# danielzgtg/TTS.cpp

Measured on AMD Instinct MI355X. Metric: audio-sec/wall-sec (RTF^-1), Parler-TTS-mini v1 Q4_K AR decode + DAC decode, higher is better.
Workload: dtype q4_K weights x q8_K activations (int dot, f32 combine); DAC f16 im2col x f32 weights, f64 accumulate

## Files before the change

### include/tts_hip.h

```cpp
#ifndef TTS_HIP_H
#define TTS_HIP_H

#include <stddef.h>
#include <stdint.h>

#ifdef __cplusplus
extern "C" {
#endif

#define TTS_MAX_DIMS 4
#define TTS_MAX_SRC 4
#define TTS_MAX_OP_PARAMS 16
#define TTS_MAX_NAME 64

enum tts_type {
    TTS_TYPE_F32 = 0,
    TTS_TYPE_F16 = 1,
    TTS_TYPE_Q4_0 = 2,
    TTS_TYPE_Q4_1 = 3,
    TTS_TYPE_Q5_0 = 6,
    TTS_TYPE_Q5_1 = 7,
    TTS_TYPE_Q8_0 = 8,
    TTS_TYPE_Q8_1 = 9,
    TTS_TYPE_Q4_K = 12,
// ... 168 lines not shown
    TTS_HIP_OPT_ATTN_PV16 = 15,
    TTS_HIP_OPT_GEMV_PREQUANT = 21,
    TTS_HIP_OPT_GEMV_KRELAY = 22,
    TTS_HIP_OPT_ATTN_KS = 23,
    TTS_HIP_OPT_ATTN_PV8 = 24,
    TTS_HIP_OPT_GEMV_KRELAY_LOOP = 26,
    TTS_HIP_OPT_GEMV_Q80_PRO = 27,
    TTS_HIP_OPT_GEMV_Q80_SLAB = 28,
    TTS_HIP_OPT_GEMV_Q80_RW = 29,
    TTS_HIP_OPT_GEMM_Q8_STAGED = 30,
    TTS_HIP_OPT_GEMV_KR_INKERNEL = 31,
    TTS_HIP_OPT_GEMV_F32_WIDE = 32,
    TTS_HIP_OPT_ATTN_PV_MP = 33,
    TTS_HIP_OPT_GEMM_KR_INKERNEL = 35,
    TTS_HIP_OPT_GEMM_KR_CT2 = 36,
    TTS_HIP_OPT_GEMM_KR_NW = 34,
    TTS_HIP_OPT_GEMV_NW_MIN = 25,
    TTS_HIP_OPT_GEMM_KR_XCD = 38,
    TTS_HIP_OPT_GEMM_KR_CP = 39,
    TTS_HIP_OPT_GEMM_KR_WALK = 40,
    TTS_HIP_OPT_GEMM_PF = 41,
    TTS_HIP_OPT_GEMM_PF_NW = 42,
    TTS_HIP_OPT_ATTN_ONE = 43,
    TTS_HIP_OPT_COALESCE = 37,
};
enum tts_fuse_bits {
    TTS_FUSE_LN = 1, TTS_FUSE_GROUP = 2, TTS_FUSE_KV = 4, TTS_FUSE_EPI = 8, TTS_FUSE_HEADS = 16, TTS_FUSE_ATTN = 32,
    TTS_FUSE_LSTM = 64,
    TTS_FUSE_SNAKE = 128,
    TTS_FUSE_EMBED = 256,
    TTS_FUSE_CONV = 512,
    TTS_FUSE_ADAIN = 1024,
    TTS_FUSE_XATTN = 2048,
    TTS_FUSE_MCPY = 4096,
    TTS_FUSE_CONTREAD = 8192
};
int tts_hip_set_option(tts_hip_backend_t backend, int option, int value);
int tts_hip_attn_decode(tts_hip_backend_t backend, const tts_tensor * q, const tts_tensor * k, const tts_tensor * v,
                        const float * mask, int64_t mbs, float scale, float * out, float * out2, const int64_t * koff,
                        const int64_t * voff, const int64_t * moff, const int32_t * pseq);
int tts_hip_coalesce_stats(int device, int64_t * out, int n);
void tts_hip_coalesce_set_wait(int us);
int tts_hip_coalesce_enable(int on);
#define TTS_HIP_HOOK_FAULT_WEIGHT_SET 1
int tts_hip_test_hook(int hook, int value);
int tts_hip_install_crash_handler(void);
// ... 3 lines not shown
typedef struct tts_sampling {
    float temperature;
    float top_p;
    float repetition_penalty;
    int32_t top_k;
    int32_t do_sample;
    int32_t pad_;
    uint64_t seed;
} tts_sampling;
void tts_sampling_default(tts_sampling * cfg);
uint32_t tts_sampler_call_seed(uint64_t seed, int32_t stream, int64_t call);
int tts_sampler_sample(const tts_sampling * cfg, const float * logits, int32_t NH, int32_t V, uint32_t call_seed, int32_t * last,
                       int32_t * count, int32_t * out);
int tts_hip_sample_step(tts_hip_backend_t backend, const float * logits, int32_t B, int32_t NH, int32_t V, const tts_sampling * cfg,
                        int64_t call, int32_t * rep_state, int32_t step, int32_t bos, int32_t eos, int32_t * eos_seen, int32_t * hist,
                        int32_t * next);
int tts_sampling_device_ok(const tts_sampling * cfg, int32_t V);
int tts_hip_counters(tts_hip_backend_t backend, int64_t * out, int n);

int tts_hip_gemv(tts_hip_backend_t backend, int type, const void * w, const float * x, float * y,
                 int64_t K, int64_t N, int64_t M);
int tts_hip_gemv_ex(tts_hip_backend_t backend, int type, const void * w, const float * x, float * y,
                    int64_t K, int64_t N, int64_t M, int32_t wflags);

typedef struct tts_backend_iface {
    void * ctx;
    const char * name;
    void * (*alloc)(void * ctx, size_t size);
    void (*free)(void * ctx, void * ptr);
    int (*set)(void * ctx, void * dst, const void * src, size_t size);
    int (*set_tensor)(void * ctx, tts_tensor * t, const void * src);
    int (*get)(void * ctx, void * dst, const void * src, size_t size);
    int (*memset)(void * ctx, void * dst, int value, size_t size);
    int (*compute)(void * ctx, tts_tensor * const * nodes, int n_nodes);
    int (*synchronize)(void * ctx);
    int (*prepare)(void * ctx, tts_tensor * const * nodes, int n_nodes, int slot);
    int (*launch)(void * ctx, int slot);
    int (*set_async)(void * ctx, void * dst, const void * src, size_t size);
    int (*copy)(void * ctx, void * dst, const void * src, size_t size);
    int (*greedy_step)(void * ctx, const float * logits, int B, int NH, int V, int step, int bos, int eos, int32_t * eos_seen,
                       int32_t * hist, int32_t * next);
    int (*sample_step)(void * ctx, const float * logits, int B, int NH, int V, const tts_sampling * cfg, int64_t call, int32_t * rep_state,
                       int step, int bos, int eos, int32_t * eos_seen, int32_t * hist, int32_t * next);
} tts_backend_iface;

int tts_hip_backend_iface(tts_hip_backend_t backend, tts_backend_iface * out);
// ... 7 lines not shown
```

### tts.cpp_amd/csrc/backend.hip

```cpp
#include <cmath>
#include <atomic>
#include <cstring>
#include <map>
#include <mutex>
#include <thread>

#include "hip_internal.h"
#include <hip/hip_ext.h>

#include <dlfcn.h>
#include <execinfo.h>
#include <fcntl.h>
#include <signal.h>
#include <unistd.h>

using namespace tts;


static void build_gelu_table(uint16_t * t) {
    const float GELU_COEF_A = 0.044715f;
    const float SQRT_2_OVER_PI = 0.79788456080286535587989211986876f;
    for (int i = 0; i < 65536; ++i) {
        const float x = fp16_to_fp32_host((uint16_t)i);
        const float g = 0.5f * x * (1.0f + tanhf(SQRT_2_OVER_PI * x * (1.0f + GELU_COEF_A * x * x)));
// ... 716 lines not shown
        case TTS_HIP_OPT_GEMV_Q80_SLAB: be->gemv_q80_slab = value != 0; return 0;
        case TTS_HIP_OPT_GEMV_KR_INKERNEL:
            if (value < 0) return TTS_STATUS_BAD_ARG;
            be->gemv_kr_ink = value;
            return 0;
        case TTS_HIP_OPT_GEMM_Q8_STAGED:
            if (value < 0 || value > 2) return TTS_STATUS_BAD_ARG;
            be->gemm_q8_staged = value;
            return 0;
        case TTS_HIP_OPT_GEMV_Q80_RW:
            if (value < 0 || value > 32 || (value & (value - 1))) return TTS_STATUS_BAD_ARG;
            be->gemv_q80_rw = value;
            return 0;
        case TTS_HIP_OPT_ATTN_KS: be->attn_ks = value; return 0;
        case TTS_HIP_OPT_GEMV_NW_MIN: be->gemv_nw_min = value; return 0;
        case TTS_HIP_OPT_ATTN_PV8: be->attn_pv8 = value != 0; return 0;
        case TTS_HIP_OPT_GEMM_KR_CT2: be->gemm_kr_ct2 = value != 0; return 0;
        case TTS_HIP_OPT_GEMM_KR_INKERNEL: be->gemm_kr_ink = value < 0 ? 0 : value; return 0;
        case TTS_HIP_OPT_ATTN_PV_MP: be->attn_pv_mp = value == 2 ? 2 : value != 0; return 0;
        case TTS_HIP_OPT_ATTN_ONE:
            if (value < 0 || value > 2) return TTS_STATUS_BAD_ARG;
            be->attn_one = value;
            return 0;
        case TTS_HIP_OPT_GEMM_KR_NW: be->gemm_kr_nw = value == 8 ? 8 : 4; return 0;
        case TTS_HIP_OPT_GEMM_Q8: be->gemm_q8 = value != 0; return 0;
        case TTS_HIP_OPT_CU_PARTITION: {
            const int count = value & 0xFF, index = (value >> 8) & 0xFF;
            const bool inter = (value >> 16) & 1;
            hipSetDevice(be->device);
            TTS_HIP_CHECK(hipStreamSynchronize(be->stream));
            hipStream_t ns = nullptr;
            if (count <= 1) {
                TTS_HIP_CHECK(hipStreamCreateWithFlags(&ns, hipStreamNonBlocking));
                be->cus = be->cu_total;
            } else {
                if (index >= count) return TTS_STATUS_BAD_ARG;
                std::vector<uint32_t> mask((be->cu_total + 31) / 32, 0u);
                const int per = be->cu_total / count;
                int n = 0;
                for (int c = 0; c < be->cu_total; ++c) {
                    const bool on = inter ? (c % count == index) : (c / per == index && c < per * count);
                    if (on) mask[c / 32] |= 1u << (c % 32), ++n;
                }
                if (hipExtStreamCreateWithCUMask(&ns, (uint32_t)mask.size(), mask.data()) != hipSuccess) return TTS_STATUS_FAILED;
                be->cus = n;
            }
// ... 113 lines not shown
```

### tts.cpp_amd/csrc/coalesce.hip

```cpp
#include <algorithm>
#include <atomic>
#include <chrono>
#include <condition_variable>
#include <cstring>
#include <map>
#include <mutex>
#include <thread>
#include <unordered_map>
#include <unordered_set>

#include "hip_internal.h"

namespace tts {
namespace {

using Clock = std::chrono::steady_clock;

struct Req {
    tts_hip_backend * be = nullptr;
    tts_tensor * const * nodes = nullptr;
    int n = 0;
    uint64_t sig = 0;
    int64_t count = 0;
    bool taken = false, done = false;
// ... 134 lines not shown
            for (int d = 0; d < 4; ++d) mix((uint64_t)t->src[0]->ne[d]);
    }
    return (h ^ (h2 * 0x94D049BB133111EBull)) | 1;
}

void copy_options(tts_hip_backend * d, const tts_hip_backend * s) {
    d->fusion = s->fusion;
    d->attn_split_minp = s->attn_split_minp;
    d->attn_ks = s->attn_ks;
    d->attn_pv_mp = s->attn_pv_mp;
    d->attn_one = s->attn_one;
    d->attn_pv8 = s->attn_pv8;
    d->attn_pv_uv16 = s->attn_pv_uv16;
    d->attn_fused_minp = s->attn_fused_minp;
    d->gemv_unique = s->gemv_unique;
    d->gemm_q8 = s->gemm_q8;
    d->bgemm_f32 = s->bgemm_f32;
    d->gemv_f32_wide = s->gemv_f32_wide;
    d->gemm_kr_nw = s->gemm_kr_nw;
    d->gemv_ks_tiles = s->gemv_ks_tiles;
    d->gemv_mf_prequant = s->gemv_mf_prequant;
    d->gemv_kr = s->gemv_kr;
    d->gemv_kr_loop = s->gemv_kr_loop;
    d->gemv_q80_pro = s->gemv_q80_pro;
    d->gemv_q80_slab = s->gemv_q80_slab;
    d->gemv_q80_rw = s->gemv_q80_rw;
    d->gemm_q8_staged = s->gemm_q8_staged;
    d->gemv_kr_ink = s->gemv_kr_ink;
    d->gemm_kr_ct2 = s->gemm_kr_ct2;
    d->gemm_kr_xcd = s->gemm_kr_xcd;
    d->gemm_kr_cp = s->gemm_kr_cp;
    d->gemm_kr_ink = s->gemm_kr_ink;
    d->gemv_nw_min = s->gemv_nw_min;
    d->gemv_mf_rsplit = s->gemv_mf_rsplit;
    d->profile_gemv = s->profile_gemv;
}

__global__ void k_ne_bytes(const uint4 * __restrict__ a, const uint4 * __restrict__ b, size_t n16, const uint8_t * __restrict__ ta,
                           const uint8_t * __restrict__ tb, size_t tail, int * flag) {
    bool ne = false;
    for (size_t i = (size_t)blockIdx.x * blockDim.x + threadIdx.x; i < n16; i += (size_t)gridDim.x * blockDim.x) {
        const uint4 x = a[i], y = b[i];
        ne |= x.x != y.x || x.y != y.y || x.z != y.z || x.w != y.w;
    }
    if (blockIdx.x == 0)
        for (size_t i = threadIdx.x; i < tail; i += blockDim.x) ne |= ta[i] != tb[i];
// ... 362 lines not shown
```

### tts.cpp_amd/csrc/graph_exec.hip

```cpp
#include <algorithm>
#include <cstring>
#include <deque>
#include <unordered_map>
#include <vector>

#include <array>

#include "hip_internal.h"
#include <chrono>

using namespace tts;

namespace tts {
void launch_kv_prefetch(tts_hip_backend * be, hipStream_t st, const TD & t, int pdim, int blocks);
void launch_gemv_q4K_xattn(tts_hip_backend * be, const GemvJob & j, const XAttnArgs & a);
void launch_attn_decode(tts_hip_backend * be, const TD & q, const TD & k, const TD & v, const float * mask, float scale,
                        float * out, int hd, int P, int H, int n, int B, float * out2, int64_t obs = -1, int64_t mbs = 0,
                        const int64_t * koff = nullptr, const int64_t * voff = nullptr, const int64_t * moff = nullptr,
                        const int * pseq = nullptr);
void launch_layernorm(tts_hip_backend * be, const tts_tensor * dst, const tts_tensor * x, const float * w, const float * b,
                      float eps, bool rms);
}

namespace {
// ... 2820 lines not shown
            if (!keep) be->aq.src = nullptr;
        }
    }
    if (pf_pending >= 0) TTS_HIP_CHECK(hipStreamWaitEvent(be->stream, be->pf_join, 0));
    if (be->bat) {
        if (n_sc > 0) {
            hipLaunchKernelGGL(k_co_scatter, dim3(4, (unsigned)n_sc), dim3(256), 0, be->stream, (const int64_t *)be->co_tab + sc_off, n_sc);
            TTS_HIP_CHECK(hipGetLastError());
            co_readback(be, sc_host, n_sc);
        }
        be->bat->comap = nullptr;
    }
    return 0;
}
}

extern "C" int tts_hip_gemv(tts_hip_backend_t be, int type, const void * w, const float * x, float * y, int64_t K, int64_t N,
                            int64_t M) {
    return tts_hip_gemv_ex(be, type, w, x, y, K, N, M, 0);
}

extern "C" int tts_hip_gemv_ex(tts_hip_backend_t be, int type, const void * w, const float * x, float * y, int64_t K, int64_t N,
                               int64_t M, int32_t wflags) {
    if (!be) return TTS_STATUS_BAD_ARG;
    if ((wflags & TTS_FLAG_TILED) && (type != TTS_TYPE_Q4_K || N % 4)) return TTS_STATUS_BAD_ARG;
    if (type == TTS_TYPE_Q4_K && K % 256) return TTS_STATUS_BAD_ARG;
    if (type == TTS_TYPE_Q8_0 && K % 32) return TTS_STATUS_BAD_ARG;
    if (type != TTS_TYPE_Q4_K && type != TTS_TYPE_Q8_0 && type != TTS_TYPE_F16 && type != TTS_TYPE_F32) return TTS_STATUS_UNSUPPORTED;
    if ((type == TTS_TYPE_F32 || type == TTS_TYPE_F16) && K % 4) return TTS_STATUS_BAD_ARG;
    hipSetDevice(be->device);
    GemvJob j;
    j.wtype = type;
    j.K = K;
    j.N = N;
    j.M = M;
    j.w_row_bytes = (int64_t)tts_row_size(type, K);
    j.W[0] = (const uint8_t *)w;
    j.Y[0] = y;
    j.ycs[0] = N;
    j.yrs[0] = 1;
    j.x = x;
    j.xcs = K;
    const bool q80pro = type == TTS_TYPE_Q8_0 && K % QK_K == 0 && M <= 8 && be->gemv_q80_pro;
    if (type == TTS_TYPE_Q4_K || q80pro) {
        j.pro = PRO_QUANT;
        j.tiled = (wflags & TTS_FLAG_TILED) ? 1 : 0;
        if ((uintptr_t)x & 15) {
            if ((size_t)(4 * K * M) > be->scratch_size) return TTS_STATUS_ALLOC_FAILED;
            launch_copy_cols(be, (float *)be->scratch, x, K, K, M);
            be->aq.src = nullptr;
            j.x = (const float *)be->scratch;
        }
    } else if (type != TTS_TYPE_F32) {
        if (act_quant_bytes(type, K, M) > be->scratch_size) return TTS_STATUS_ALLOC_FAILED;
        launch_quantize_act(be, type, x, K, K, M, j.aq);
    } else {
        j.aq.vtype = TTS_TYPE_F32;
    }
    be->aq.src = nullptr;
    launch_gemv_job(be, j);
    return 0;
}
```

### tts.cpp_amd/csrc/hip_internal.h

```cpp
#pragma once

#include <hip/hip_fp16.h>
#include <hip/hip_runtime.h>

#include <cstdio>
#include <cstdlib>
#include <atomic>
#include <deque>
#include <mutex>
#include <unordered_map>
#include <tuple>
#include <vector>

#include "common.h"

#define TTS_HIP_CHECK(expr)                                                                          \
    do {                                                                                             \
        hipError_t err_ = (expr);                                                                    \
        if (err_ != hipSuccess) {                                                                    \
            fprintf(stderr, "%s:%d: HIP error %s: %s\n", __FILE__, __LINE__, #expr, hipGetErrorString(err_)); \
            abort();                                                                                 \
        }                                                                                            \
    } while (0)

// ... 151 lines not shown
    int64_t xcs = 0;
    ActQuant aq;
    int pro = 0;
    int tiled = 0;
    int hetero = 0;
    int64_t roff[GEMV_MAX_MATS + 1] = {};
    int32_t rep_mat = -1, yrg = 0, nrep = 0;
    int64_t yrgs = 0, yrep = 0;
    int dbg = 0;
    const float * lnw = nullptr;
    const float * lnb = nullptr;
    float eps = 0.f;
    int rms = 0;
    float * lnout = nullptr;
    int64_t locs = 0;
    const char * bq = nullptr;
    int64_t bq_bytes = 0;
    int64_t bq_tile = 0;
    int32_t bq_slot = 0;
    unsigned long long * ts = nullptr;
    const int64_t * yoff = nullptr;
    int32_t yoff_mats = 0, yoff_ld = 0;
    int32_t xcd_cols = 0;
};
__host__ __device__ inline int64_t job_roff(const GemvJob & j, int m) { return j.hetero ? j.roff[m] : (int64_t)m * j.N; }
__host__ __device__ inline int64_t job_rows(const GemvJob & j) { return job_roff(j, j.nmat); }
#ifdef TTS_PHASE_TS
#define TTS_TS(job, k)                                                                                            \
    do {                                                                                                          \
        if ((job).ts && (threadIdx.x & 63) == 0)                                                                  \
            (job).ts[((((size_t)blockIdx.z * gridDim.y + blockIdx.y) * gridDim.x + blockIdx.x) * (blockDim.x >> 6) + \
                      (threadIdx.x >> 6)) * 8 +                                                                   \
                     (k)] = __builtin_amdgcn_s_memrealtime();                                                     \
    } while (0)
#else
#define TTS_TS(job, k) \
    do {               \
    } while (0)
#endif
enum { PRO_QUANT = 1, PRO_LN = 2, PRO_COPY = 3 };
struct XAttnArgs {
    TD k, v;
    const float * mask = nullptr;
    float scale = 1.f;
    float * out = nullptr;
    float * out2 = nullptr;
    int P = 0, H = 0, B = 0;
// ... 78 lines not shown
    size_t attn_floats = 0;
    int attn_split_minp = 128;
    int attn_ks = 2;
    int attn_pv_mp = 1;
    int attn_one = 1;
    int attn_pv8 = 0;
    int attn_pv_uv16 = 0;
    int attn_fused_minp = 0;
    unsigned long long * argmax_keys = nullptr;
    unsigned * argmax_counts = nullptr;
    int64_t q4k_tile_bytes = 4 << 20;
    int gemv_dbg = 0;
    int gemv_unique = 1;
    int gemm_q8 = 1;
    int64_t cus = 256;
    int cu_total = 256;
    int bgemm_f32 = 1;
    int gemv_f32_wide = 1;
    int gemm_kr_nw = 4;
    int64_t gemv_ks_tiles = 256;
    int gemv_mf_prequant = 1;
    int gemv_kr = 1;
    int gemv_kr_loop = 1;
    int gemv_q80_pro = 1;
    int gemv_q80_slab = 1;
    int gemv_q80_rw = 0;
    int gemm_q8_staged = 2;
    int64_t gemv_kr_ink = 0;
    int gemm_kr_walk = 0;
    int gemm_pf = 64;
    int gemm_pf_nw = 4;
    int gemm_kr_cp = 0;
    int gemm_kr_xcd = 0;
    int gemm_kr_ct2 = 0;
    int64_t gemm_kr_ink = 0;
    int gemv_nw_min = 0;
    int gemv_mf_rsplit = 1;
    int64_t q4k_dual_bytes = 1 << 20;
    void * sample_cand = nullptr;
    size_t sample_cand_size = 0;
    int kv_prefetch_minp = 0;
    int kv_prefetch_blocks = 128;
    hipStream_t pf_stream = nullptr;
    hipEvent_t pf_fork = nullptr, pf_join = nullptr;
    uint8_t * pin = nullptr;
    size_t pin_size = 0, pin_head = 0;
// ... 189 lines not shown
```

### tts.cpp_amd/csrc/k_gemv.hip

```cpp
#include "hip_internal.h"
#include <hip/hip_ext.h>

#include <atomic>
#include <type_traits>

#ifndef TTS_GEMV_EARLY16
#define TTS_GEMV_EARLY16 1
#endif

namespace tts {

__device__ __forceinline__ float dev_fp16_to_fp32(uint16_t h) {
    return __half2float(__ushort_as_half(h));
}

__device__ __forceinline__ int dev_nearest_int(float f) {
    const float val = __fadd_rn(f, 12582912.f);
    const int i = __float_as_int(val);
    return (i & 0x007fffff) - 0x00400000;
}

__global__ __launch_bounds__(256) void k_quantize_q8_K(const float * __restrict__ x, int64_t xcs, int64_t K,
                                                       int8_t * __restrict__ qs, float * __restrict__ dout,
                                                       int32_t * __restrict__ s32) {
// ... 83 lines not shown
    const int m = blockIdx.y;
    const int64_t i = (int64_t)blockIdx.x * blockDim.x + threadIdx.x;
    if (i < K) out[m * K + i] = __float2half_rn(x[m * xcs + i]);
}

__device__ __forceinline__ void q4k_scale_min(const uint8_t * q, int j, int & sc, int & mn) {
    if (j < 4) {
        sc = q[j] & 63;
        mn = q[j + 4] & 63;
    } else {
        sc = (q[j + 4] & 0xF) | ((q[j - 4] >> 6) << 4);
        mn = (q[j + 4] >> 4) | ((q[j] >> 6) << 4);
    }
}

__device__ __forceinline__ size_t al16(size_t n) { return (n + 15) & ~(size_t)15; }

__device__ __forceinline__ int xcd_contiguous(int b, int n) {
    const int x = b & 7, q = n >> 3, r = n & 7;
    return x * q + (x < r ? x : r) + (b >> 3);
}


template <int MC>
__device__ __forceinline__ void gemv_store(const GemvJob & j, int mat, int64_t row, int m, float v) {
    if (j.epi == EPI_GELU) {
        if (v <= -10.0f) v = 0.0f;
        else if (v < 10.0f) v = __half2float(__ushort_as_half(j.gelu[__half_as_ushort(__float2half_rn(v))]));
    } else if (j.epi == EPI_ADD) {
        v = __fadd_rn(v, j.res[m * j.rcs + row]);
    } else if (j.epi == EPI_SILU_MUL) {
        v = __fmul_rn(dev_silu(j.res[m * j.rcs + row]), v);
    }
    float * const Y = j.Y[mat] + ((j.yoff_mats >> mat) & 1 ? j.yoff[mat * j.yoff_ld + m] : 0);
    const int64_t ycs = j.ycs[mat], yrs = j.yrs[mat];
    if (mat == j.rep_mat) {
        const int64_t g = row / j.yrg;
        float * y = Y + m * ycs + g * j.yrgs + (row - g * j.yrg) * yrs;
        for (int k = 0; k < j.nrep; ++k) y[k * j.yrep] = v;
        return;
    }
    Y[m * ycs + row * yrs] = v;
}

__device__ __forceinline__ void q8k_quant16(const float (&v)[16], int lane, int (&q)[16], float & d, int & s) {
    float lax = 0.f, lval = 0.f;
#pragma unroll
    for (int e = 0; e < 16; ++e) {
        const float a = fabsf(v[e]);
        const bool gt = a > lax;
        lax = gt ? a : lax;
        lval = gt ? v[e] : lval;
    }
    unsigned mx = __float_as_uint(lax);
    mx = max(mx, (unsigned)dpp_i32<DPP_XOR1>((int)mx));
    mx = max(mx, (unsigned)dpp_i32<DPP_XOR2>((int)mx));
// ... 844 lines not shown
                    qb[bf][u][l] = ld((const uint32_t *)(bp + 16 + (l + 4) * 16 + kg * 4));
                }
            }
        } else {
            const uint8_t * wt = j.W[mat] + (row >> 2) * nb * 576;
            const int ri = (int)(row & 3);
#pragma unroll
            for (int u = 0; u < BPW; ++u) {
                const uint8_t * bp = wt + (int64_t)min(w * BPW + u, nb - 1) * 576;
                hd[bf][u] = ld((const u32x4 *)(bp + ri * 16));
                qa[bf][u] = ld((const u32x4 *)(bp + 64 + ((kg * 2) * 4 + ri) * 16));
                qb[bf][u] = ld((const u32x4 *)(bp + 64 + ((kg * 2 + 1) * 4 + ri) * 16));
            }
        }
        TTS_PIN_LOADS();
    };
    auto load_w = [&](auto BUF, int64_t t) __attribute__((always_inline)) {
        if (!LOOP && CTW == 1 && j.xcd_cols && gridDim.y > 1) load_w_pol(BUF, std::true_type{}, t);
        else load_w_pol(BUF, std::false_type{}, t);
    };
    using B0 = std::integral_constant<int, 0>;
    using B1 = std::integral_constant<int, LOOP ? 1 : 0>;
    int64_t t = tx;
    if constexpr (PRO == PRO_COPY) {
        const int nck = (int)((ntile * bqb) >> 10);
        for (int i = wave; i < nck; i += nw)
            __builtin_amdgcn_global_load_lds(gptr(bqt + (size_t)i * 1024 + lane * 16),
                                             (__attribute__((address_space(3))) void *)(smem + (size_t)i * 1024), 16, 0, 0);
        TTS_PIN_LOADS();
        load_w(B0{}, t);
    } else {
        auto first = [&]() __attribute__((always_inline)) { load_w(B0{}, t); };
        ProOv ov;
        ov.col0 = c0;
        ov.mcols = M;
        q4k_prologue<PRO, 16, true, decltype(first)>(j, nb, nullptr, xd_s, nullptr, b16, sbs, first, ov);
    }
    TTS_TS(j, 1);
    __syncthreads();
    TTS_TS(j, 2);

    f2v tp[BPW][8][2], tq[BPW][2];
    auto terms = [&](auto BUF) __attribute__((always_inline)) {
        constexpr int bf = decltype(BUF)::value;
#pragma unroll
        for (int u = 0; u < BPW; ++u) {
            const int b = min(w * BPW + u, nb - 1);
            const u32x4 h = hd[bf][u];
            const uint32_t sc_lo = h.y & 0x3F3F3F3Fu, mn_lo = h.z & 0x3F3F3F3Fu;
            const uint32_t sc_hi = (h.w & 0x0F0F0F0Fu) | ((h.y >> 2) & 0x30303030u);
            const uint32_t mn_hi = ((h.w >> 4) & 0x0F0F0F0Fu) | ((h.z >> 2) & 0x30303030u);
            const uint32_t sw = (kg < 2 ? sc_lo : sc_hi) >> ((kg & 1) * 16);
            const _Float16 s0 = (_Float16)(float)(sw & 0xFF), s1 = (_Float16)(float)((sw >> 8) & 0xFF);
            const f16x2 S0 = {s0, s0}, S1 = {s1, s1};
            const _Float16 o0 = (_Float16)(-1024.f * (float)(sw & 0xFF)), o1 = (_Float16)(-1024.f * (float)((sw >> 8) & 0xFF));
// ... 87 lines not shown
        float tot[4];
        if (w == nwt - 1) {
#pragma unroll
            for (int q = 0; q < 4; ++q) {
                tot[q] = sumf[q >> 1][q & 1];
#pragma unroll
                for (int l = 0; l < 8; ++l) tot[q] = __fadd_rn(tot[q], sums[l][q >> 1][q & 1]);
            }
        }
        if constexpr (SW) {
            float * xg = relay + 2 * 64 * 36;
            if (w == nwt - 1 && sub == 0) *(float4 *)(xg + lane * 4) = make_float4(tot[0], tot[1], tot[2], tot[3]);
            __syncthreads();
            if (w == nwt - 1 && sub == 1) {
                const float4 g4 = *(const float4 *)(xg + lane * 4);
                const float gv[4] = {g4.x, g4.y, g4.z, g4.w};
#pragma unroll
                for (int q = 0; q < 4; ++q) {
                    const int64_t flat = tt * 16 + 4 * kg + q;
                    if (r < M && flat < NR) j.Y[0][(c0 + r) * j.ycs[0] + flat * j.yrs[0]] = __fmul_rn(dev_silu(gv[q]), tot[q]);
                }
            }
        } else if (w == nwt - 1) {
            const int mat = tile_mat(tt);
            const int64_t row0 = tile_row0(tt, mat);
            const int64_t rows_m = job_roff(j, mat + 1) - job_roff(j, mat);
#pragma unroll
            for (int q = 0; q < 4; ++q) {
                const int64_t rr = row0 + 4 * kg + q;
                if (r < M && rr < rows_m) gemv_store<8>(j, mat, rr, c0 + r, tot[q]);
            }
        }
    };

    if constexpr (LOOP) {
        const int64_t G = gridDim.x;
        for (; t < T; t += 2 * G) {
            terms(B0{});
            load_w(B1{}, t + G);
            TTS_TS(j, 3);
            relay_store(t);
            TTS_TS(j, 4);
            __syncthreads();
            if (t + G >= T) break;
            terms(B1{});
            load_w(B0{}, t + 2 * G);
            relay_store(t + G);
            __syncthreads();
        }
    } else {
        terms(B0{});
        TTS_TS(j, 3);
        relay_store(t);
        TTS_TS(j, 4);
        if constexpr (CTW > 1) {
            for (int k = 1; k < ntile; ++k) {
                __syncthreads();
                c0 = 16 * (ct0 + k);
                M = min(16, (int)j.M - c0);
                nslot = M * nb + 1;
                b16 = (_Float16 *)(smem + (size_t)k * bqb);
                sbs = b16 + (size_t)nslot * QK_K;
                xd_s = (float *)(sbs + (size_t)nslot * 16);
                cc = r < M ? r : M - 1;
                terms(B0{});
                relay_store(t);
            }
        }
    }
    TTS_TS(j, 5);
}

constexpr int PF_RS = 2;
constexpr int PF_SLOT = QK_K + 8;
template <int NB, bool LANE, int NW = 4>
__global__ __launch_bounds__(64 * NW) void k_gemm_q4K_pf(GemvJob j) {
// ... 995 lines not shown
            ji.bq = nullptr;
            ji.bq_bytes = bq;
            if (launch_q4k_kr(be, ji)) continue;
        }
        if (be->gemv_mf_prequant && !j.dbg && (size_t)(bq + 4 * j.K * j.M) <= be->scratch_size) {
            j.bq = be->scratch + be->scratch_size - bq;
            j.bq_bytes = bq;
            const dim3 qg((unsigned)((nb + 3) / 4), (unsigned)j.M);
            if (j.pro == PRO_LN) hipLaunchKernelGGL(k_quant_mf<PRO_LN>, qg, dim3(64), 0, be->stream, j);
            else hipLaunchKernelGGL(k_quant_mf<PRO_QUANT>, qg, dim3(64), 0, be->stream, j);
            TTS_HIP_CHECK(hipGetLastError());
            j.pro = PRO_COPY;
            j.lnout = nullptr;
            if (!launch_q4k_kr(be, j)) launch_q4k_mf_pro<PRO_COPY, 16>(be, j);
            continue;
        }
        if (j.pro == PRO_LN) launch_q4k_mf_pro<PRO_LN, 16>(be, j);
        else launch_q4k_mf_pro<PRO_QUANT, 16>(be, j);
    }
}

static size_t q4k_kr_lds(int64_t bq_bytes, bool sw) { return (size_t)((bq_bytes + 15) & ~15) + (sw ? 2 * 64 * 36 * 4 + 64 * 16 : 64 * 36 * 4); }
template <int BPW, bool SW, int NWT, bool LANE = false, bool LOOP = false, int PRO = PRO_COPY, int CTW = 1, bool CP = false>
static void launch_q4k_kr_t(tts_hip_backend * be, const GemvJob & j, unsigned gx, unsigned gy = 1) {
    if constexpr (PRO == PRO_COPY && CTW == 1 && !CP) {
        if (j.pro == PRO_LN) return launch_q4k_kr_t<BPW, SW, NWT, LANE, LOOP, PRO_LN>(be, j, gx, gy);
        if (j.pro == PRO_QUANT) return launch_q4k_kr_t<BPW, SW, NWT, LANE, LOOP, PRO_QUANT>(be, j, gx, gy);
    }
    if constexpr (SW && !LOOP && BPW <= 3 && CTW == 1) {
        if (be->gemv_kr_loop && gx > (unsigned)be->cus && gy == 1) {
            launch_q4k_kr_t<BPW, SW, NWT, LANE, true, PRO>(be, j, (unsigned)be->cus, gy);
            return;
        }
    }
    static std::atomic<uint32_t> attr_done{0};
    set_lds_attr_once(attr_done, be->device, (const void *)k_gemv_q4K_kr<BPW, SW, NWT, LANE, LOOP, PRO, CTW, CP>);
    const size_t lds = q4k_kr_lds((CP ? 2 : CTW) * (j.bq_tile ? j.bq_tile : j.bq_bytes), SW || CP);
    const dim3 blk(64 * NWT * ((SW || CP) ? 2 : 1));
    if (be->profile_gemv) {
        hipEvent_t e0, e1;
        profile_pair(be, e0, e1);
        hipExtLaunchKernelGGL((k_gemv_q4K_kr<BPW, SW, NWT, LANE, LOOP, PRO, CTW, CP>), dim3(gx, gy), blk, (uint32_t)lds, be->stream, e0, e1, 0u, j);
        profile_push(be, e0, e1, gemv_bytes(j), TTS_TYPE_Q4_K);
        return;
    }
    hipLaunchKernelGGL((k_gemv_q4K_kr<BPW, SW, NWT, LANE, LOOP, PRO, CTW, CP>), dim3(gx, gy), blk, lds, be->stream, j);
}

static size_t q4k_pf_lds(int64_t nb) { return (size_t)((((16 * nb + 1) * (2 * PF_SLOT + 32 + 4)) + 1023) & ~(int64_t)1023); }
template <int NB, bool LANE, int NW>
static void launch_q4k_pf_nw(tts_hip_backend * be, const GemvJob & j, unsigned gy) {
    static std::atomic<uint32_t> attr_done{0};
    set_lds_attr_once(attr_done, be->device, (const void *)k_gemm_q4K_pf<NB, LANE, NW>);
    const unsigned gx = (unsigned)((job_rows(j) / 16 + NW * PF_RS - 1) / (NW * PF_RS));
    hipLaunchKernelGGL((k_gemm_q4K_pf<NB, LANE, NW>), dim3(gx, gy), dim3(64 * NW), (uint32_t)q4k_pf_lds(NB), be->stream, j);
}
template <int NB, bool LANE>
static void launch_q4k_pf_t(tts_hip_backend * be, const GemvJob & j, unsigned gy) {
    if (be->gemm_pf_nw == 8) launch_q4k_pf_nw<NB, LANE, 8>(be, j, gy);
    else launch_q4k_pf_nw<NB, LANE, 4>(be, j, gy);
// ... 568 lines not shown
```

### tts.cpp_amd/ttship/__init__.py

```python
import ctypes
import os
import pathlib

_HERE = pathlib.Path(__file__).resolve().parent
PKG_ROOT = _HERE.parent
REPO_ROOT = PKG_ROOT.parent
LIB_PATH = PKG_ROOT / "lib" / "libtts_hip.so"

F32, F16, Q4_0, Q8_0, Q4_K, Q8_K, I32 = 0, 1, 2, 8, 12, 15, 26
PROF_ATTN = 39

OPS = ["NONE", "DUP", "ADD", "SUB", "MUL", "DIV", "SQR", "SQRT", "SIN", "COS", "SUM_ROWS", "REPEAT",
       "CONCAT", "NORM", "RMS_NORM", "MUL_MAT", "SCALE", "CPY", "CONT", "RESHAPE", "VIEW", "PERMUTE",
       "TRANSPOSE", "GET_ROWS", "SOFT_MAX", "ROPE", "CLAMP", "CONV_TRANSPOSE_1D", "IM2COL", "UPSCALE",
       "PAD", "LEAKY_RELU", "UNARY", "CUMSUM", "MOD", "ROUND", "STFT", "ISTFT", "MAP_CUSTOM3", "MAP_CUSTOM2"]
OP = {n: i for i, n in enumerate(OPS)}
FUSE = {"LN": 1, "GROUP": 2, "KV": 4, "EPI": 8, "HEADS": 16, "ATTN": 32, "LSTM": 64, "SNAKE": 128, "EMBED": 256, "CONV": 512, "ADAIN": 1024, "XATTN": 2048, "MCPY": 4096, "CONTREAD": 8192}
FUSE_ALL = sum(FUSE.values())
UNARY = {"ABS": 0, "NEG": 1, "TANH": 2, "RELU": 3, "SIGMOID": 4, "GELU": 5, "SILU": 6, "EXP": 7}

OPT = {"FUSION": 0, "PROFILE_GEMV": 1, "GRAPHS": 2, "CONV_F32ACC": 3, "CONVT_LDS": 4, "ATTN_SPLIT": 5, "KV_PREFETCH": 6, "KV_PREFETCH_BLOCKS": 7, "Q4K_TILE_BYTES": 8, "GEMV_DEBUG": 10, "GEMV_UNIQUE": 11, "CONV_SPLIT": 12, "GEMV_KS": 13, "ATTN_FUSED": 14, "ATTN_PV16": 15, "Q4K_DUAL_BYTES": 16, "GEMV_RSPLIT": 17, "GEMM_Q8": 18, "BGEMM_F32": 19, "CU_PARTITION": 20, "GEMV_PREQUANT": 21, "GEMV_KRELAY": 22, "ATTN_KS": 23, "ATTN_PV8": 24, "GEMV_NW_MIN": 25, "GEMV_KRELAY_LOOP": 26, "GEMV_Q80_PRO": 27, "GEMV_Q80_SLAB": 28, "GEMV_Q80_RW": 29, "GEMM_Q8_STAGED": 30, "GEMV_KR_INKERNEL": 31, "GEMV_F32_WIDE": 32, "ATTN_PV_MP": 33, "GEMM_KR_NW": 34, "GEMM_KR_INKERNEL": 35, "GEMM_KR_CT2": 36, "COALESCE": 37, "GEMM_KR_XCD": 38, "GEMM_KR_CP": 39, "GEMM_KR_WALK": 40, "GEMM_PF": 41, "GEMM_PF_NW": 42, "ATTN_ONE": 43}
ATTN_SPLIT_DEFAULT = 128
ATTN_ONE_DEFAULT = 1
ATTN_FUSED_ON = 128

TYPE_SIZE = {F32: 4, F16: 2, Q4_K: 144, Q8_0: 34, I32: 4}
BLCK_SIZE = {F32: 1, F16: 1, Q4_K: 256, Q8_0: 32, I32: 1}


class TtsTensor(ctypes.Structure):
    pass


TtsTensor._fields_ = [
    ("type", ctypes.c_int32),
    ("op", ctypes.c_int32),
    ("ne", ctypes.c_int64 * 4),
    ("nb", ctypes.c_uint64 * 4),
    ("op_params", ctypes.c_int32 * 16),
    ("src", ctypes.POINTER(TtsTensor) * 4),
    ("view_src", ctypes.POINTER(TtsTensor)),
    ("view_offs", ctypes.c_uint64),
    ("data", ctypes.c_void_p),
    ("flags", ctypes.c_int32),
    ("pad_", ctypes.c_int32),
    ("name", ctypes.c_char * 64),
# ... 245 lines not shown
        "tts_op_name": (ctypes.c_char_p, [ctypes.c_int]),
        "tts_hip_device_count": (ctypes.c_int, []),
        "tts_hip_backend_init": (vp, [ctypes.c_int]),
        "tts_hip_backend_free": (None, [vp]),
        "tts_hip_backend_name": (ctypes.c_char_p, [vp]),
        "tts_hip_buffer_alloc": (vp, [vp, sz]),
        "tts_hip_buffer_free": (None, [vp, vp]),
        "tts_hip_buffer_alignment": (sz, []),
        "tts_hip_tensor_set": (ctypes.c_int, [vp, vp, vp, sz]),
        "tts_hip_tensor_get": (ctypes.c_int, [vp, vp, vp, sz]),
        "tts_hip_tensor_copy": (ctypes.c_int, [vp, vp, vp, sz]),
        "tts_hip_copy_stream": (ctypes.c_int, [vp, vp, vp, sz]),
        "tts_hip_memset": (ctypes.c_int, [vp, vp, ctypes.c_int, sz]),
        "tts_hip_synchronize": (ctypes.c_int, [vp]),
        "tts_hip_supports_op": (ctypes.c_int, [ctypes.POINTER(TtsTensor)]),
        "tts_hip_graph_compute": (ctypes.c_int, [vp, ctypes.POINTER(ctypes.POINTER(TtsTensor)), ctypes.c_int]),
        "tts_hip_set_option": (ctypes.c_int, [vp, ctypes.c_int, ctypes.c_int]),
        "tts_hip_attn_decode": (ctypes.c_int, [vp, ctypes.POINTER(TtsTensor), ctypes.POINTER(TtsTensor), ctypes.POINTER(TtsTensor), vp,
                                               i64, ctypes.c_float, vp, vp, vp, vp, vp, vp]),
        "tts_hip_gemv_stats": (ctypes.c_int, [vp, ctypes.c_int, ctypes.POINTER(ctypes.c_double), ctypes.POINTER(i64),
                                              ctypes.POINTER(ctypes.c_double), ctypes.c_int]),
        "tts_hip_gemv": (ctypes.c_int, [vp, ctypes.c_int, vp, vp, vp, i64, i64, i64]),
        "tts_hip_gemv_ex": (ctypes.c_int, [vp, ctypes.c_int, vp, vp, vp, i64, i64, i64, i32]),
        "tts_hip_counters": (ctypes.c_int, [vp, ctypes.POINTER(i64), ctypes.c_int]),
        "tts_hip_coalesce_stats": (ctypes.c_int, [ctypes.c_int, ctypes.POINTER(i64), ctypes.c_int]),
        "tts_hip_coalesce_set_wait": (None, [ctypes.c_int]),
        "tts_hip_coalesce_enable": (ctypes.c_int, [ctypes.c_int]),
        "tts_hip_test_hook": (ctypes.c_int, [ctypes.c_int, ctypes.c_int]),
        "tts_hip_install_crash_handler": (ctypes.c_int, []),
        "tts_parler_n_weights": (i32, [vp]),
        "tts_dia_n_weights": (i32, [vp]),
        "tts_dia_weight": (u64, [vp, i32, ctypes.c_char_p, u64, ctypes.POINTER(i64), ctypes.POINTER(i32), vp, u64]),
        "tts_parler_weight": (u64, [vp, i32, ctypes.c_char_p, u64, ctypes.POINTER(i64), ctypes.POINTER(i32), vp, u64]),
        "tts_orpheus_n_weights": (i32, [vp]),
        "tts_orpheus_weight": (u64, [vp, i32, ctypes.c_char_p, u64, ctypes.POINTER(i64), ctypes.POINTER(i32), vp, u64]),
        "tts_dac_n_weights": (i32, [vp]),
        "tts_dac_weight": (u64, [vp, i32, ctypes.c_char_p, u64, ctypes.POINTER(i64), ctypes.POINTER(i32), vp, u64]),
        "tts_sampling_default": (None, [ctypes.POINTER(Sampling)]),
        "tts_parler_set_sampling": (None, [vp, ctypes.POINTER(Sampling)]),
        "tts_parler_set_position": (ctypes.c_int, [vp, i32]),
        "tts_dia_set_sampling": (None, [vp, ctypes.POINTER(Sampling)]),
        "tts_orpheus_set_sampling": (None, [vp, ctypes.POINTER(Sampling)]),
        "tts_sampler_call_seed": (ctypes.c_uint32, [ctypes.c_uint64, i32, i64]),
        "tts_sampler_sample": (ctypes.c_int, [ctypes.POINTER(Sampling), vp, i32, i32, ctypes.c_uint32, vp, vp, vp]),
        "tts_hip_sample_step": (ctypes.c_int, [vp, vp, i32, i32, i32, ctypes.POINTER(Sampling), i64, vp, i32, i32, i32, vp, vp, vp]),
        "tts_hip_greedy_step": (ctypes.c_int, [vp, vp, i32, i32, i32, i32, i32, i32, vp, vp, vp]),
# ... 1097 lines not shown
```

Baseline: 108.7.

## Prefetch residual and fold K-relay reduction tail in Q4_K relay GEMV

Result: faster. 110.3, median of 6 (+1.5%).

```diff
diff --git a/include/tts_hip.h b/include/tts_hip.h
--- a/include/tts_hip.h
+++ b/include/tts_hip.h
@@ -214,6 +214,7 @@
     TTS_HIP_OPT_GEMM_PF = 41,
     TTS_HIP_OPT_GEMM_PF_NW = 42,
     TTS_HIP_OPT_ATTN_ONE = 43,
+    TTS_HIP_OPT_GEMV_KR_TAIL = 44,
     TTS_HIP_OPT_COALESCE = 37,
 };
 enum tts_fuse_bits {
@@ -263,6 +264,8 @@
                  int64_t K, int64_t N, int64_t M);
 int tts_hip_gemv_ex(tts_hip_backend_t backend, int type, const void * w, const float * x, float * y,
                     int64_t K, int64_t N, int64_t M, int32_t wflags);
+int tts_hip_gemv_res(tts_hip_backend_t backend, int type, const void * w, const float * x, float * y, const float * res,
+                     int64_t K, int64_t N, int64_t M, int32_t wflags);
 
 typedef struct tts_backend_iface {
     void * ctx;
diff --git a/tts.cpp_amd/csrc/backend.hip b/tts.cpp_amd/csrc/backend.hip
--- a/tts.cpp_amd/csrc/backend.hip
+++ b/tts.cpp_amd/csrc/backend.hip
@@ -762,6 +762,10 @@
             if (value < 0 || value > 2) return TTS_STATUS_BAD_ARG;
             be->attn_one = value;
             return 0;
+        case TTS_HIP_OPT_GEMV_KR_TAIL:
+            if (value < 0 || value > 4) return TTS_STATUS_BAD_ARG;
+            be->gemv_kr_tail = value;
+            return 0;
         case TTS_HIP_OPT_GEMM_KR_NW: be->gemm_kr_nw = value == 8 ? 8 : 4; return 0;
         case TTS_HIP_OPT_GEMM_Q8: be->gemm_q8 = value != 0; return 0;
         case TTS_HIP_OPT_CU_PARTITION: {
diff --git a/tts.cpp_amd/csrc/coalesce.hip b/tts.cpp_amd/csrc/coalesce.hip
--- a/tts.cpp_amd/csrc/coalesce.hip
+++ b/tts.cpp_amd/csrc/coalesce.hip
@@ -180,6 +180,7 @@
     d->gemv_mf_prequant = s->gemv_mf_prequant;
     d->gemv_kr = s->gemv_kr;
     d->gemv_kr_loop = s->gemv_kr_loop;
+    d->gemv_kr_tail = s->gemv_kr_tail;
     d->gemv_q80_pro = s->gemv_q80_pro;
     d->gemv_q80_slab = s->gemv_q80_slab;
     d->gemv_q80_rw = s->gemv_q80_rw;
diff --git a/tts.cpp_amd/csrc/graph_exec.hip b/tts.cpp_amd/csrc/graph_exec.hip
--- a/tts.cpp_amd/csrc/graph_exec.hip
+++ b/tts.cpp_amd/csrc/graph_exec.hip
@@ -2866,6 +2866,11 @@
 
 extern "C" int tts_hip_gemv_ex(tts_hip_backend_t be, int type, const void * w, const float * x, float * y, int64_t K, int64_t N,
                                int64_t M, int32_t wflags) {
+    return tts_hip_gemv_res(be, type, w, x, y, nullptr, K, N, M, wflags);
+}
+
+extern "C" int tts_hip_gemv_res(tts_hip_backend_t be, int type, const void * w, const float * x, float * y, const float * res,
+                                int64_t K, int64_t N, int64_t M, int32_t wflags) {
     if (!be) return TTS_STATUS_BAD_ARG;
     if ((wflags & TTS_FLAG_TILED) && (type != TTS_TYPE_Q4_K || N % 4)) return TTS_STATUS_BAD_ARG;
     if (type == TTS_TYPE_Q4_K && K % 256) return TTS_STATUS_BAD_ARG;
@@ -2885,6 +2890,11 @@
     j.yrs[0] = 1;
     j.x = x;
     j.xcs = K;
+    if (res) {
+        j.epi = EPI_ADD;
+        j.res = res;
+        j.rcs = N;
+    }
     const bool q80pro = type == TTS_TYPE_Q8_0 && K % QK_K == 0 && M <= 8 && be->gemv_q80_pro;
     if (type == TTS_TYPE_Q4_K || q80pro) {
         j.pro = PRO_QUANT;
diff --git a/tts.cpp_amd/csrc/hip_internal.h b/tts.cpp_amd/csrc/hip_internal.h
--- a/tts.cpp_amd/csrc/hip_internal.h
+++ b/tts.cpp_amd/csrc/hip_internal.h
@@ -197,7 +197,10 @@
     const int64_t * yoff = nullptr;
     int32_t yoff_mats = 0, yoff_ld = 0;
     int32_t xcd_cols = 0;
-};
+    int32_t kr_tail = 0;
+};
+enum { KR_TAIL_RES = 1, KR_TAIL_FOLD = 2, KR_TAIL_BESIDE = 4 };
+constexpr int KR_FOLD_BYTES = 4 * 4 * (2 * 64 * 16 + 64 * 4);
 __host__ __device__ inline int64_t job_roff(const GemvJob & j, int m) { return j.hetero ? j.roff[m] : (int64_t)m * j.N; }
 __host__ __device__ inline int64_t job_rows(const GemvJob & j) { return job_roff(j, j.nmat); }
 #ifdef TTS_PHASE_TS
@@ -322,6 +325,7 @@
     int gemv_mf_prequant = 1;
     int gemv_kr = 1;
     int gemv_kr_loop = 1;
+    int gemv_kr_tail = 1;
     int gemv_q80_pro = 1;
     int gemv_q80_slab = 1;
     int gemv_q80_rw = 0;
diff --git a/tts.cpp_amd/csrc/k_gemv.hip b/tts.cpp_amd/csrc/k_gemv.hip
--- a/tts.cpp_amd/csrc/k_gemv.hip
+++ b/tts.cpp_amd/csrc/k_gemv.hip
@@ -129,6 +129,7 @@
 }
 
 
+__device__ __forceinline__ void gemv_put(const GemvJob & j, int mat, int64_t row, int m, float v);
 template <int MC>
 __device__ __forceinline__ void gemv_store(const GemvJob & j, int mat, int64_t row, int m, float v) {
     if (j.epi == EPI_GELU) {
@@ -139,6 +140,13 @@
     } else if (j.epi == EPI_SILU_MUL) {
         v = __fmul_rn(dev_silu(j.res[m * j.rcs + row]), v);
     }
+    gemv_put(j, mat, row, m, v);
+}
+__device__ __forceinline__ void gemv_store_res(const GemvJob & j, int mat, int64_t row, int m, float v, float rv, bool pre) {
+    if (pre) gemv_put(j, mat, row, m, __fadd_rn(v, rv));
+    else gemv_store<8>(j, mat, row, m, v);
+}
+__device__ __forceinline__ void gemv_put(const GemvJob & j, int mat, int64_t row, int m, float v) {
     float * const Y = j.Y[mat] + ((j.yoff_mats >> mat) & 1 ? j.yoff[mat * j.yoff_ld + m] : 0);
     const int64_t ycs = j.ycs[mat], yrs = j.yrs[mat];
     if (mat == j.rep_mat) {
@@ -1029,6 +1037,30 @@
     using B0 = std::integral_constant<int, 0>;
     using B1 = std::integral_constant<int, LOOP ? 1 : 0>;
     int64_t t = tx;
+    constexpr bool TAIL = !SW && !LOOP && CTW == 1 && !CP;
+    const bool res_pre = TAIL && j.epi == EPI_ADD && (j.kr_tail & KR_TAIL_RES);
+    int tmat = 0;
+    int64_t trow0 = 0, trows = 0;
+    const float * rp[4] = {};
+    if constexpr (TAIL) {
+        tmat = tile_mat(t);
+        trow0 = tile_row0(t, tmat);
+        trows = job_roff(j, tmat + 1) - job_roff(j, tmat);
+        const float * const base = res_pre ? j.res + (int64_t)(c0 + cc) * j.rcs : (const float *)j.W[tmat];
+#pragma unroll
+        for (int q = 0; q < 4; ++q) {
+            const int64_t rr = trow0 + 4 * kg + q < trows ? trow0 + 4 * kg + q : trows - 1;
+            rp[q] = base + (res_pre ? rr : 0);
+        }
+    }
+    float rv[4] = {0.f, 0.f, 0.f, 0.f};
+    auto load_res = [&]() __attribute__((always_inline)) {
+        if constexpr (TAIL) {
+#pragma unroll
+            for (int q = 0; q < 4; ++q) rv[q] = *gptr(rp[q]);
+            TTS_PIN_LOADS();
+        }
+    };
     if constexpr (PRO == PRO_COPY) {
         const int nck = (int)((ntile * bqb) >> 10);
         for (int i = wave; i < nck; i += nw)
@@ -1036,8 +1068,12 @@
                                              (__attribute__((address_space(3))) void *)(smem + (size_t)i * 1024), 16, 0, 0);
         TTS_PIN_LOADS();
         load_w(B0{}, t);
+        load_res();
     } else {
-        auto first = [&]() __attribute__((always_inline)) { load_w(B0{}, t); };
+        auto first = [&]() __attribute__((always_inline)) {
+            load_w(B0{}, t);
+            load_res();
+        };
         ProOv ov;
         ov.col0 = c0;
         ov.mcols = M;
@@ -1171,15 +1207,54 @@
                 }
             }
         } else if (w == nwt - 1) {
-            const int mat = tile_mat(tt);
-            const int64_t row0 = tile_row0(tt, mat);
-            const int64_t rows_m = job_roff(j, mat + 1) - job_roff(j, mat);
+            const int mat = TAIL ? tmat : tile_mat(tt);
+            const int64_t row0 = TAIL ? trow0 : tile_row0(tt, mat);
+            const int64_t rows_m = TAIL ? trows : job_roff(j, mat + 1) - job_roff(j, mat);
 #pragma unroll
             for (int q = 0; q < 4; ++q) {
                 const int64_t rr = row0 + 4 * kg + q;
-                if (r < M && rr < rows_m) gemv_store<8>(j, mat, rr, c0 + r, tot[q]);
-            }
-        }
+                if (r < M && rr < rows_m) gemv_store_res(j, mat, rr, c0 + r, tot[q], rv[q], res_pre);
+            }
+        }
+    };
+
+    auto fold_store = [&](int64_t tt) __attribute__((always_inline)) {
+        const bool beside = j.kr_tail & KR_TAIL_BESIDE;
+        float * const fb = beside ? relay : (float *)smem;
+        constexpr int FQ = 2 * 64 * 4 + 64;
+        if (!beside) __syncthreads();
+#pragma unroll
+        for (int q = 0; q < 4; ++q) {
+            float * const p = fb + (size_t)(w * 4 + q) * FQ;
+            const int hq = q >> 1, e = q & 1;
+            *(float4 *)(p + lane * 4) = make_float4(tp[0][0][hq][e], tp[0][1][hq][e], tp[0][2][hq][e], tp[0][3][hq][e]);
+            *(float4 *)(p + 256 + lane * 4) = make_float4(tp[0][4][hq][e], tp[0][5][hq][e], tp[0][6][hq][e], tp[0][7][hq][e]);
+            p[512 + lane] = tq[0][hq][e];
+        }
+        __syncthreads();
+        float4 pa[4], pb[4];
+        float pq[4];
+#pragma unroll
+        for (int b = 0; b < 4; ++b) {
+            const float * const p = fb + (size_t)(b * 4 + w) * FQ;
+            pa[b] = *(const float4 *)(p + lane * 4);
+            pb[b] = *(const float4 *)(p + 256 + lane * 4);
+            pq[b] = p[512 + lane];
+        }
+        float sums[8] = {0.f, 0.f, 0.f, 0.f, 0.f, 0.f, 0.f, 0.f}, sumf = 0.f;
+#pragma unroll
+        for (int b = 0; b < 4; ++b) {
+            const float pl[8] = {pa[b].x, pa[b].y, pa[b].z, pa[b].w, pb[b].x, pb[b].y, pb[b].z, pb[b].w};
+#pragma unroll
+            for (int l = 0; l < 8; ++l) sums[l] = __fadd_rn(sums[l], pl[l]);
+            sumf = __fsub_rn(sumf, pq[b]);
+        }
+        float tot = sumf;
+#pragma unroll
+        for (int l = 0; l < 8; ++l) tot = __fadd_rn(tot, sums[l]);
+        const int64_t rr = trow0 + 4 * kg + w;
+        const float rw = w == 0 ? rv[0] : w == 1 ? rv[1] : w == 2 ? rv[2] : rv[3];
+        if (r < M && rr < trows) gemv_store_res(j, tmat, rr, c0 + r, tot, rw, res_pre);
     };
 
     if constexpr (LOOP) {
@@ -1200,7 +1275,12 @@
     } else {
         terms(B0{});
         TTS_TS(j, 3);
-        relay_store(t);
+        if constexpr (TAIL && BPW == 1 && NWT == 4) {
+            if ((j.kr_tail & KR_TAIL_FOLD) && nb == 4) fold_store(t);
+            else relay_store(t);
+        } else {
+            relay_store(t);
+        }
         TTS_TS(j, 4);
         if constexpr (CTW > 1) {
             for (int k = 1; k < ntile; ++k) {
@@ -2242,7 +2322,10 @@
 
 static size_t q4k_kr_lds(int64_t bq_bytes, bool sw) { return (size_t)((bq_bytes + 15) & ~15) + (sw ? 2 * 64 * 36 * 4 + 64 * 16 : 64 * 36 * 4); }
 template <int BPW, bool SW, int NWT, bool LANE = false, bool LOOP = false, int PRO = PRO_COPY, int CTW = 1, bool CP = false>
-static void launch_q4k_kr_t(tts_hip_backend * be, const GemvJob & j, unsigned gx, unsigned gy = 1) {
+static void launch_q4k_kr_t(tts_hip_backend * be, const GemvJob & job, unsigned gx, unsigned gy = 1) {
+    static const int tail_bits[5] = {0, KR_TAIL_RES | KR_TAIL_FOLD, KR_TAIL_RES | KR_TAIL_FOLD | KR_TAIL_BESIDE, KR_TAIL_RES, KR_TAIL_FOLD};
+    GemvJob j = job;
+    j.kr_tail = tail_bits[be->gemv_kr_tail];
     if constexpr (PRO == PRO_COPY && CTW == 1 && !CP) {
         if (j.pro == PRO_LN) return launch_q4k_kr_t<BPW, SW, NWT, LANE, LOOP, PRO_LN>(be, j, gx, gy);
         if (j.pro == PRO_QUANT) return launch_q4k_kr_t<BPW, SW, NWT, LANE, LOOP, PRO_QUANT>(be, j, gx, gy);
@@ -2255,7 +2338,13 @@
     }
     static std::atomic<uint32_t> attr_done{0};
     set_lds_attr_once(attr_done, be->device, (const void *)k_gemv_q4K_kr<BPW, SW, NWT, LANE, LOOP, PRO, CTW, CP>);
-    const size_t lds = q4k_kr_lds((CP ? 2 : CTW) * (j.bq_tile ? j.bq_tile : j.bq_bytes), SW || CP);
+    size_t lds = q4k_kr_lds((CP ? 2 : CTW) * (j.bq_tile ? j.bq_tile : j.bq_bytes), SW || CP);
+    if constexpr (!SW && !LOOP && CTW == 1 && !CP && BPW == 1 && NWT == 4) {
+        if ((j.kr_tail & KR_TAIL_FOLD) && j.K == 4 * QK_K) {
+            const size_t ops = lds - 64 * 36 * 4;
+            lds = (j.kr_tail & KR_TAIL_BESIDE) ? ops + KR_FOLD_BYTES : std::max(ops, (size_t)KR_FOLD_BYTES);
+        }
+    }
     const dim3 blk(64 * NWT * ((SW || CP) ? 2 : 1));
     if (be->profile_gemv) {
         hipEvent_t e0, e1;
diff --git a/tts.cpp_amd/ttship/__init__.py b/tts.cpp_amd/ttship/__init__.py
--- a/tts.cpp_amd/ttship/__init__.py
+++ b/tts.cpp_amd/ttship/__init__.py
@@ -19,9 +19,10 @@
 FUSE_ALL = sum(FUSE.values())
 UNARY = {"ABS": 0, "NEG": 1, "TANH": 2, "RELU": 3, "SIGMOID": 4, "GELU": 5, "SILU": 6, "EXP": 7}
 
-OPT = {"FUSION": 0, "PROFILE_GEMV": 1, "GRAPHS": 2, "CONV_F32ACC": 3, "CONVT_LDS": 4, "ATTN_SPLIT": 5, "KV_PREFETCH": 6, "KV_PREFETCH_BLOCKS": 7, "Q4K_TILE_BYTES": 8, "GEMV_DEBUG": 10, "GEMV_UNIQUE": 11, "CONV_SPLIT": 12, "GEMV_KS": 13, "ATTN_FUSED": 14, "ATTN_PV16": 15, "Q4K_DUAL_BYTES": 16, "GEMV_RSPLIT": 17, "GEMM_Q8": 18, "BGEMM_F32": 19, "CU_PARTITION": 20, "GEMV_PREQUANT": 21, "GEMV_KRELAY": 22, "ATTN_KS": 23, "ATTN_PV8": 24, "GEMV_NW_MIN": 25, "GEMV_KRELAY_LOOP": 26, "GEMV_Q80_PRO": 27, "GEMV_Q80_SLAB": 28, "GEMV_Q80_RW": 29, "GEMM_Q8_STAGED": 30, "GEMV_KR_INKERNEL": 31, "GEMV_F32_WIDE": 32, "ATTN_PV_MP": 33, "GEMM_KR_NW": 34, "GEMM_KR_INKERNEL": 35, "GEMM_KR_CT2": 36, "COALESCE": 37, "GEMM_KR_XCD": 38, "GEMM_KR_CP": 39, "GEMM_KR_WALK": 40, "GEMM_PF": 41, "GEMM_PF_NW": 42, "ATTN_ONE": 43}
+OPT = {"FUSION": 0, "PROFILE_GEMV": 1, "GRAPHS": 2, "CONV_F32ACC": 3, "CONVT_LDS": 4, "ATTN_SPLIT": 5, "KV_PREFETCH": 6, "KV_PREFETCH_BLOCKS": 7, "Q4K_TILE_BYTES": 8, "GEMV_DEBUG": 10, "GEMV_UNIQUE": 11, "CONV_SPLIT": 12, "GEMV_KS": 13, "ATTN_FUSED": 14, "ATTN_PV16": 15, "Q4K_DUAL_BYTES": 16, "GEMV_RSPLIT": 17, "GEMM_Q8": 18, "BGEMM_F32": 19, "CU_PARTITION": 20, "GEMV_PREQUANT": 21, "GEMV_KRELAY": 22, "ATTN_KS": 23, "ATTN_PV8": 24, "GEMV_NW_MIN": 25, "GEMV_KRELAY_LOOP": 26, "GEMV_Q80_PRO": 27, "GEMV_Q80_SLAB": 28, "GEMV_Q80_RW": 29, "GEMM_Q8_STAGED": 30, "GEMV_KR_INKERNEL": 31, "GEMV_F32_WIDE": 32, "ATTN_PV_MP": 33, "GEMM_KR_NW": 34, "GEMM_KR_INKERNEL": 35, "GEMM_KR_CT2": 36, "COALESCE": 37, "GEMM_KR_XCD": 38, "GEMM_KR_CP": 39, "GEMM_KR_WALK": 40, "GEMM_PF": 41, "GEMM_PF_NW": 42, "ATTN_ONE": 43, "GEMV_KR_TAIL": 44}
 ATTN_SPLIT_DEFAULT = 128
 ATTN_ONE_DEFAULT = 1
+GEMV_KR_TAIL_DEFAULT = 1
 ATTN_FUSED_ON = 128
 
 TYPE_SIZE = {F32: 4, F16: 2, Q4_K: 144, Q8_0: 34, I32: 4}
@@ -313,6 +314,7 @@
                                               ctypes.POINTER(ctypes.c_double), ctypes.c_int]),
         "tts_hip_gemv": (ctypes.c_int, [vp, ctypes.c_int, vp, vp, vp, i64, i64, i64]),
         "tts_hip_gemv_ex": (ctypes.c_int, [vp, ctypes.c_int, vp, vp, vp, i64, i64, i64, i32]),
+        "tts_hip_gemv_res": (ctypes.c_int, [vp, ctypes.c_int, vp, vp, vp, vp, i64, i64, i64, i32]),
         "tts_hip_counters": (ctypes.c_int, [vp, ctypes.POINTER(i64), ctypes.c_int]),
         "tts_hip_coalesce_stats": (ctypes.c_int, [ctypes.c_int, ctypes.POINTER(i64), ctypes.c_int]),
         "tts_hip_coalesce_set_wait": (None, [ctypes.c_int]),
```
